# eladb3/SViT

Measured on AMD Instinct MI355X. Metric: clips/sec (fwd+bwd) SViT 16x224^2 bf16, higher is better.
Workload: dtype bf16; 1 GPU; SViT 16x224^2, 8 clips/GPU, 4 object tokens/frame, fwd+CE+bwd+clip+AdamW; global_batch=8, parallelism=dp1, ranks_seen=1, forced_dp=False, launch=hip-graph replay, input=fp32 clips, resident in the replayed step's input buffers, hip_library=svit_amd/lib/libsvit_hip.so

## Files before the change

### include/svit_hip.h

```cpp
#ifndef SVIT_HIP_H
#define SVIT_HIP_H
#include <stdint.h>
#ifdef __cplusplus
extern "C" {
#endif

#define SVIT_HEAD_DIM 96

int svit_version(void);
const char* svit_arch(void);

enum {
  SVIT_EPI_BF16 = 0,
  SVIT_EPI_GELU = 1,
  SVIT_EPI_RESID = 2,
  SVIT_EPI_F32 = 3,
  SVIT_EPI_DGELU = 4,
  SVIT_EPI_RELQ = 5
};
typedef struct {
  const void* A; int32_t lda;
  const void* W; int32_t ldw;
  const float* bias;
  void* out; int32_t ldo;
// ... 8 lines not shown
  int32_t relq_extra, relq_rows;
  float relq_scale;
} svit_gemm_args;
int svit_gemm_nt(const svit_gemm_args* args, void* stream);
int svit_gemm_tn(const void* A, int lda, const void* B, int ldb, float* dW, int lddw,
                 int M, int N, int K, int splits, float* dbias ,
                 void* stream);
#define SVIT_TN_GROUP_MAX 16
typedef struct {
  const void* A; const void* B; float* dW; float* dbias;
  int32_t lda, ldb, lddw, M, N, K;
} svit_tn_problem;
int svit_gemm_tn_grouped(const svit_tn_problem* probs, int count, void* stream);
int svit_gemm_tn_grouped_ex(const svit_tn_problem* probs, int count, int ordered, void* stream);
int svit_gemm_tn_grouped_slab(const svit_tn_problem* probs, int count, float* workspace,
                              int64_t workspace_floats, void* stream);
int64_t svit_gemm_tn_grouped_workspace(const svit_tn_problem* probs, int count);
int svit_colsum_bf16(const void* A, int lda, float* out, int M, int N, void* stream);

int svit_cast_f32_bf16(const float* src, void* dst, int64_t n, void* stream);
int svit_table_interp(const float* M, int rows, int J, const float* tables, float* out32, void* out16, void* stream);
typedef struct svit_table_interp_job {
  const float* M;
  const float* tables;
  float* out32;
  void* out16;
  int32_t rows, J;
} svit_table_interp_job;
int svit_table_interp_batched(const svit_table_interp_job* jobs_dev, int n_jobs, int max_rows, void* stream);
int svit_transpose_cast_batched(const float* src_base, void* dst_base, const int64_t* table,
                                int n_mats, int max_tiles, void* stream);
int svit_transpose_bf16_batched(const void* src_base, void* dst_base, const int64_t* table,
                                int n_mats, int max_tiles, void* stream);
int svit_pad_cast_rows(const float* src, void* dst, int R, int C, int ldd, void* stream);
int svit_scale_cast(const float* src, void* dst, const float* row_scale, int rows_per_sample,
                    int64_t rows, int cols, int gather_L, int gather_N, int gather_off,
                    void* stream);

int svit_reduce_defer(int on, void* stream);
int svit_reduce_flush(void* stream);
int svit_reduce_reset(void* stream);

int svit_layernorm_fwd(const float* x, const float* gamma, const float* beta, void* y_bf16,
                       float* y_f32, float* mean, float* rstd, int64_t rows, int C, float eps,
                       void* stream);
int svit_layernorm_bwd(const void* dy , int dy_is_bf16,
                       const float* x, const float* gamma, const float* mean,
                       const float* rstd, const float* dres, float* dx, void* dx_bf16,
                       const float* row_scale, int rows_per_sample, float* dgamma,
                       float* dbeta, int64_t rows, int C, float* workspace,
                       int64_t workspace_floats, void* stream);

int svit_im2col_patch(const float* video, void* cols, int B, int T, int H, int W, void* stream);
int svit_im2col_patch_u8(const uint8_t* frames, int64_t frames_bytes, const void* lut,
                         const int32_t* crops, void* cols, int B, int T, int Hs, int Ws, int S,
                         void* stream);
int svit_mixup_clips(float* x, const void* mix, int B, int planes, int H, int W, void* stream);
int svit_im2col_patch_u8_mix(const uint8_t* frames, int64_t frames_bytes, const float* lut_f32,
                             const int32_t* crops, const void* mix, void* cols, int B, int T, int Hs,
                             int Ws, int S, void* stream);
int svit_fill_special_tokens(float* x, const float* cls, const float* objq, const float* pos_t,
                             int B, int N, int L, int Tx, int O, int C, int add_pos, void* stream);
int svit_special_token_grads(const float* dx, float* g_cls, float* g_obj, float* g_pos, int B, int N,
                             int L, int Tx, int O, int C, int add_pos, void* stream);

typedef struct {
  const void* qkv; int32_t which;
  const float* conv_w;
  const float* gamma; const float* beta;
  void* out; int32_t ld_out;
  void* pre; float* mean; float* rstd;
  int32_t B, heads, T, H, W, n_obj;
  int32_t stride_hw;
  int32_t mode;
  float eps;
  float out_scale;
  const void* relq_R; const int32_t* relq_map; int32_t relq_lpad; float relq_scale;
} svit_pool_args;
int svit_pool_ln_fwd(const svit_pool_args* a, void* stream);

typedef struct {
  const void* d_main; int32_t main_is_f32; int32_t ld_main;
  const void* d_res; const void* d_extra;
  const void* pre; const float* mean; const float* rstd; const float* gamma;
  void* dpre; float* dgamma; float* dbeta;
  int32_t B, heads, Nout;
  float* workspace; int64_t workspace_floats;
  int32_t main_parts; int64_t main_part_stride;
  int32_t extra_is_bf16;
} svit_pool_ln_bwd_args;
int svit_pool_ln_bwd(const svit_pool_ln_bwd_args* a, void* stream);
typedef struct {
  const void* dpre; const float* conv_w; void* dqkv; int32_t which;
  int32_t B, heads, T, H, W, n_obj, stride_hw;
} svit_pool_dgrad_args;
typedef struct {
  const void* dpre; const void* qkv; int32_t which; float* dw;
  int32_t B, heads, T, H, W, n_obj, stride_hw;
  float* workspace; int64_t workspace_floats;
} svit_pool_wgrad_args;
int svit_pool_ln_fwd_qkv(const svit_pool_args* args3, void* stream);
int svit_pool_weight_sel(const float* src_base, const int64_t* src_off, uint32_t* dst, int n_tables,
                         void* stream);
int svit_pool_ln_fwd_qkv_sel(const svit_pool_args* args3, const uint32_t* const* sel3, void* stream);
int svit_pool_ln_bwd_qkv(const svit_pool_ln_bwd_args* args3, void* stream);
#ifdef SVIT_DIAG_POOL_STREAMING
// ... 127 lines not shown
```

### svit_amd/build.py

```python
import concurrent.futures
import os
import re
import subprocess
import sys

HERE = os.path.dirname(os.path.abspath(__file__))
CSRC = os.path.join(HERE, "csrc")
OUT_DIR = os.path.join(HERE, "lib")
LIB = os.path.join(OUT_DIR, "libsvit_hip.so")
SOURCES = ["gemm_nt.hip", "gemm_tn.hip", "norm.hip", "misc.hip", "pool.hip", "attn_fwd.hip", "attn_bwd.hip",
           "loss.hip", "meter.hip", "input.hip", "head.hip"]
HEADERS = ["common.h", "attn_common.h", "gemm_epilogue.h", os.path.join("..", "..", "include", "svit_hip.h")]
HIPCC = os.environ.get("HIPCC", "/opt/rocm/bin/hipcc")
FLAGS = ["--offload-arch=gfx950", "-O3", "-fPIC", "-std=c++17", "-ffast-math",
         "-fno-finite-math-only", "-fno-slp-vectorize", "-Wno-unused-result"]
TMP_DIR = os.path.join(OUT_DIR, "tmp")


_PK = re.compile(r"\s*(v_pk_(?:mul|add|fma)_f32)\s+v\[(\d+):\d+\],\s*(.*)")


def _sel(rest, name, n, default):
    m = re.search(name + r":\[([0-9,]+)\]", rest)
    v = [int(x) for x in m.group(1).split(",")] if m else []
    return v + [default] * (n - len(v))


def hazardous_packed_f32(asm_text):
    bad = []
    for ln, line in enumerate(asm_text.splitlines(), 1):
        m = _PK.match(line)
        if not m:
            continue
        rest = m.group(3).split("//")[0]
        ops = [o.strip() for o in re.split(r",\s*(?![^\[]*\])", rest.split(" op_sel")[0].split(" neg_")[0])]
        sel = _sel(rest, "op_sel", len(ops), 0) if re.search(r"op_sel:\[", rest) else [0] * len(ops)
        sel_hi = _sel(rest, "op_sel_hi", len(ops), 1)
        for i, o in enumerate(ops):
            if re.match(r"v\[(\d+):\d+\]", o) and (sel[i] == 1 or sel_hi[i] == 0):
                bad.append((ln, line.split("//")[0].strip()))
                break
    return bad


LLVM_OBJDUMP = os.environ.get("LLVM_OBJDUMP", "/opt/rocm/lib/llvm/bin/llvm-objdump")


def disassemble(lib=None):
    import shutil
    import tempfile
    lib = lib or LIB
    tmp = tempfile.mkdtemp(prefix="svit_isa_")
    try:
        cp = os.path.join(tmp, "lib.so")
        shutil.copy(lib, cp)
        r = subprocess.run([LLVM_OBJDUMP, "--offloading", cp], capture_output=True, text=True, cwd=tmp)
        if r.returncode != 0:
            raise RuntimeError("llvm-objdump --offloading failed: %s" % r.stderr[-300:])
        objs = sorted(f for f in os.listdir(tmp) if "amdgcn" in f and "gfx950" in f)
        text = []
        for f in objs:
            d = subprocess.run([LLVM_OBJDUMP, "-d", "--no-show-raw-insn", os.path.join(tmp, f)],
                               capture_output=True, text=True)
            if d.returncode != 0:
# ... 69 lines not shown
```

### svit_amd/engine.py

```python
import math

import torch

from . import arch, hip, ops
from .input import U8Clips

HD = arch.HEAD_DIM
F32, BF16 = torch.float32, torch.bfloat16
SCALE = HD ** -0.5
LOG2E = 1.4426950408889634
K_SCALE = SCALE * LOG2E


def _align(n, a=8):
    return (n + a - 1) // a * a


class FlatParams:

    def __init__(self, shapes, decay_of, device, rank_of):
        names = list(shapes)
        depth = 1 + max([int(n.split(".")[1]) for n in names if n.startswith("blocks.")] or [0])
        ranks = {n: rank_of(n, depth) for n in names}
        order = sorted(names, key=lambda n: (not decay_of(n, shapes[n]), ranks[n]))
# ... 83 lines not shown

    def sels(self, pre):
        return [self.pool_sel[self.pool_sel_index[pre + "attn.pool_%s.weight" % r]] for r in "qkv"]

    TILED_MIN_PLANE = 2048
    SLAB_MAX_PLANE = 196

    def refresh_low_precision(self):
        ops.cast_bf16(self.data, self.w16[:self.total])
        if self.pool_sel_index:
            ops.pool_weight_sel(self.data, self.pool_sel_off, self.pool_sel)
        if self.n_t:
            ops.transpose_bf16_batched(self.w16, self.wT16, self.t_table, self.n_t, 256)


def rel_sections(rows):
    off_w = _align(rows[0])
    off_t = off_w + _align(rows[1])
    return (0, off_w, off_t), _align(off_t + rows[2], 32)


def _rel_index(q_n, k_n):
    q_ratio = max(k_n / q_n, 1.0)
    k_ratio = max(q_n / k_n, 1.0)
    d = torch.arange(q_n)[:, None] * q_ratio - torch.arange(k_n)[None, :] * k_ratio
    d = d + (k_n - 1) * k_ratio
    return d.long().to(torch.int32)


def _resize_matrix(rows_have, rows_need):
    m = torch.zeros(rows_need, rows_have)
    scale = rows_have / rows_need
    for i in range(rows_need):
        pos = max((i + 0.5) * scale - 0.5, 0.0)
        i0 = min(int(math.floor(pos)), rows_have - 1)
        i1 = min(i0 + 1, rows_have - 1)
        lam = pos - i0
        m[i, i0] += 1.0 - lam
        m[i, i1] += lam
    return m


class Engine:
    def __init__(self, plan: arch.Plan, flat: FlatParams, red_group=4):
        self.plan, self.flat = plan, flat
        self.dev = flat.data.device
        self._rel_cache = {}
        self._interp_cache = {}
        self._interp_out = {}
        self.batch_interp = True
        self._relq_cache = {}
        self.fused_scatter = True
        self.patch_w16 = torch.zeros((plan.embed_dim, 448), device=self.dev, dtype=BF16)
        self._tn = []
        self.RED_GROUP = max(1, int(red_group))
        M1 = 1024 * 1024
        self._red_ws = torch.empty(self.RED_GROUP * 18 * M1, device=self.dev, dtype=F32)
        self._red_slot = 0
        self._wgrad_need, self._wgrad_big = {}, {}
        self._red_regions = {"ln2": (0, 4 * M1), "ln1": (4 * M1, 8 * M1), "pln": (8 * M1, 9 * M1),
                             "wgrad": (9 * M1, 18 * M1)}
        self._side = None
        self._side_keep = []
        self._side_active = False
        self.overlap_wgrad = False
        self.attn_q_splits = 0
        self.deterministic = False
        self.reproducible = False
        self._capture_fork = None
        self._capture_join = None

    def refresh_weights(self):
        self.flat.refresh_low_precision()
        ops.pad_cast_rows(self.flat.p("patch_embed.proj.weight").view(self.plan.embed_dim, 441),
                          self.patch_w16)

    def _rel(self, blk, q_thw, k_thw):
        key = (blk.index, q_thw, k_thw)
        ent = self._rel_cache.get(key)
        if ent is None:
            idx = [_rel_index(q_thw[1], k_thw[1]), _rel_index(q_thw[2], k_thw[2]),
                   _rel_index(q_thw[0], k_thw[0])]
            need = [2 * max(q_thw[i], k_thw[i]) - 1 for i in (1, 2, 0)]
            have = [blk.rel_sp_rows, blk.rel_sp_rows, blk.rel_t_rows]
            mats = [None if n == h else _resize_matrix(h, n).to(self.dev) for n, h in zip(need, have)]
            mcat = None
            if any(m is not None for m in mats):
                lp = (sum(need) + 95) // 96 * 96
                mcat = torch.zeros((lp, sum(have)), device=self.dev)
                r0 = c0 = 0
                for n, h, m in zip(need, have, mats):
                    mcat[r0:r0 + n, c0:c0 + h] = torch.eye(h, device=self.dev) if m is None else m
                    r0, c0 = r0 + n, c0 + h
            ent = ([t.contiguous().to(self.dev) for t in idx], mats, mcat, tuple(need))
            self._rel_cache[key] = ent
        return ent

    def _interp_tables(self, thw, save):
        if not self.batch_interp:
            self._interp_out = {}
            return
        key = (tuple(thw), bool(save))
        ent = self._interp_cache.get(key)
        if ent is None:
            entries, outs, cur = [], {}, tuple(thw)
            for blk in self.plan.blocks:
                sq, skv = blk.stride_q[1], blk.stride_kv[1]
                q_thw = (cur[0], arch.pooled(cur[1], sq), arch.pooled(cur[2], sq))
                k_thw = (cur[0], arch.pooled(cur[1], skv), arch.pooled(cur[2], skv))
                _, _, mcat, _ = self._rel(blk, q_thw, k_thw)
                if mcat is not None:
                    r32 = torch.empty((mcat.shape[0], HD), device=self.dev, dtype=F32) if save else None
                    r16 = torch.empty((mcat.shape[0], HD), device=self.dev, dtype=BF16)
                    entries.append((mcat, self.flat.rel_tables32("blocks.%d." % blk.index), r32, r16))
                    outs[blk.index] = (r32, r16)
                cur = q_thw
            jobs = ops.table_interp_jobs(entries, self.dev) if entries else None
            ent = (jobs, max((e[0].shape[0] for e in entries), default=0), outs, entries)
            self._interp_cache[key] = ent
        jobs, max_rows, outs, _ = ent
        if jobs is not None:
            ops.table_interp_batched(jobs, max_rows)
        self._interp_out = outs

    def _relq_map(self, blk, q_thw, k_thw, idx, rows_off, n_obj, extra):
        key = (blk.index, q_thw, k_thw, tuple(rows_off), n_obj, extra)
        m = self._relq_cache.get(key)
        if m is None:
            qt, qh, qw = q_thw
            kt, kh, kw = k_thw
            ih, iw, it = (t.cpu().view(n, k) for t, n, k in zip(idx, (qh, qw, qt), (kh, kw, kt)))
            Lq = qt * qh * qw
            body = torch.full((qt, qh, qw, extra), -1, dtype=torch.int32)
            body[..., :kh] = (rows_off[0] + ih).view(1, qh, 1, kh)
            body[..., kh:kh + kw] = (rows_off[1] + iw).view(1, 1, qw, kw)
            body[..., kh + kw:kh + kw + kt] = (rows_off[2] + it).view(qt, 1, 1, kt)
            m = torch.full((1 + Lq + n_obj, extra), -1, dtype=torch.int32)
            m[1:1 + Lq] = body.view(Lq, extra)
            m = m.contiguous().to(self.dev)
            self._relq_cache[key] = m
        return m

    def _tables(self, pre, mats):
        names = (pre + "attn.rel_pos_h", pre + "attn.rel_pos_w", pre + "attn.rel_pos_t")
        out = []
        for n, m in zip(names, mats):
            t = self.flat.p(n)
            out.append(t if m is None else (m @ t).contiguous())
        return out

    def forward(self, video, drop_scales=None, save=True):
        plan, f = self.plan, self.flat
        if isinstance(video, U8Clips):
            B, _, Tx = video.shape[:3]
            cols, (To, Ho, Wo) = ops.im2col_patch_u8(video)
        else:
            if video.dim() == 4:
                video = video.unsqueeze(2)
            video = video.contiguous().to(F32)
            B, _, Tx = video.shape[:3]
            cols, (To, Ho, Wo) = ops.im2col_patch(video)
        T = plan.num_frames // plan.patch_stride[0] if Tx > 1 else Tx
        if To != T:
            raise hip.SvitHipError("clip has %d frames but cfg.DATA.NUM_FRAMES=%d" % (Tx, plan.num_frames))
        L, n_obj, C = To * Ho * Wo, Tx * plan.objects, plan.embed_dim
        N = 1 + L + n_obj
        x = torch.empty((B, N, C), device=self.dev, dtype=F32)
        ops.gemm_nt(cols, self.patch_w16, f.p("patch_embed.proj.bias"), hip.EPI_F32,
                    out=x.view(B * N, C), remap=(L, N, 1))
        ops.fill_special_tokens(x, f.p("cls_token"), f.p("object_queries"),
                                f.p("pos_embed_temporal"), L, Tx, plan.objects, Tx > 1)
        st = {"B": B, "Tx": Tx, "n_obj": n_obj, "L0": L, "cols": cols if save else None,
              "blocks": []}
        thw = (T, Ho, Wo)
        self._interp_tables(thw, save)
        hip.mark("stem")
        for blk in plan.blocks:
            ds = drop_scales[blk.index] if drop_scales is not None else None
            x, thw, sv = self._block_fwd(blk, x, thw, n_obj, ds, save)
            st["blocks"].append(sv)
            hip.mark("fwd%d" % blk.index)
        y16, y32, mean, rstd = ops.layernorm_fwd(x, f.p("norm.weight"), f.p("norm.bias"),
                                                 want_f32=True, want_bf16=False, save_stats=save)
        st.update(x_last=x if save else None, mean=mean, rstd=rstd, thw=thw)
        self._interp_out = {}
        return y32, st

    def _block_fwd(self, blk, x, thw, n_obj, ds, save):
        f = self.flat
        pre = "blocks.%d." % blk.index
        B, N, C = x.shape
        Co, h = blk.dim_out, blk.heads
        sq, skv = blk.stride_q[1], blk.stride_kv[1]
        q_thw = (thw[0], arch.pooled(thw[1], sq), arch.pooled(thw[2], sq))
        k_thw = (thw[0], arch.pooled(thw[1], skv), arch.pooled(thw[2], skv))
        Nq = 1 + q_thw[0] * q_thw[1] * q_thw[2] + n_obj
        J = k_thw[0] + k_thw[1] + k_thw[2]
        DA = HD + 32 if J <= 32 else HD + 64
        if J > 64:
            raise hip.SvitHipError("key grid %s too large for the in-MFMA rel-pos bias" % (k_thw,))
        xn, _, mean1, rstd1 = ops.layernorm_fwd(x, f.p(pre + "norm1.weight"), f.p(pre + "norm1.bias"),
                                                save_stats=save)
        xn2d = xn.view(B * N, C)
        qkv = ops.gemm_nt(xn2d, f.w(pre + "attn.qkv.weight"), f.p(pre + "attn.qkv.bias"), hip.EPI_BF16)
        idx, mats, mcat, need = self._rel(blk, q_thw, k_thw)
        if mcat is None:
            tabs = self._tables(pre, mats)
            rcat, rows_off = f.rel_cat(pre)
        else:
            if blk.index in self._interp_out:
                r32, rcat = self._interp_out[blk.index]
            else:
                r32, rcat = ops.table_interp(mcat, f.rel_tables32(pre), want_f32=save)
            rows_off = (0, need[0], need[0] + need[1])
            tabs = None if r32 is None else [r32[rows_off[0]:rows_off[0] + need[0]], r32[rows_off[1]:rows_off[1] + need[1]],
                                             r32[rows_off[2]:rows_off[2] + need[2]]]
        pools = ops.pool_ln_fwd_qkv(
            qkv, [f.p(pre + "attn.pool_%s.weight" % r).view(HD, 27) for r in "qkv"],
            [f.p(pre + "attn.norm_%s.weight" % r) for r in "qkv"],
            [f.p(pre + "attn.norm_%s.bias" % r) for r in "qkv"],
            B, h, thw, n_obj, (sq, skv, skv), (DA, DA, HD), (0, 1, 0), save=save, out_scales=(1.0, K_SCALE, 1.0),
            sels=f.sels(pre) if (thw[1] * thw[2] >= f.TILED_MIN_PLANE or thw[1] * thw[2] <= f.SLAB_MAX_PLANE)
            else None,
            relq=(rcat.contiguous(), self._relq_map(blk, q_thw, k_thw, idx, rows_off, n_obj, DA - HD), LOG2E))
        qa, ka, v = pools[0][0], pools[1][0], pools[2][0]
        ctx, lse2 = ops.attn_fwd(qa, ka, v, SCALE, bias_cols=J)
# ... 6 lines not shown
        if blk.pools_q:
            skip, pool_idx = ops.maxpool_fwd(skip, thw, n_obj)
        dpa, dpm = ds if ds is not None else (None, None)
        x1 = ops.gemm_nt(ctx.view(B * Nq, Co), f.w(pre + "attn.proj.weight"), f.p(pre + "attn.proj.bias"),
                         hip.EPI_RESID, aux=skip.view(B * Nq, Co), row_scale=dpa, rows_per_sample=Nq)
        x1 = x1.view(B, Nq, Co)
        xn2, _, mean2, rstd2 = ops.layernorm_fwd(x1, f.p(pre + "norm2.weight"), f.p(pre + "norm2.bias"),
                                                 save_stats=save)
        act, dact = ops.gemm_nt(xn2.view(B * Nq, Co), f.w(pre + "mlp.fc1.weight"),
                                f.p(pre + "mlp.fc1.bias"), hip.EPI_GELU, save=save)
        x2 = ops.gemm_nt(act, f.w(pre + "mlp.fc2.weight"), f.p(pre + "mlp.fc2.bias"), hip.EPI_RESID,
                         aux=x1.view(B * Nq, Co), row_scale=dpm, rows_per_sample=Nq).view(B, Nq, Co)
        sv = None
        if save:
            sv = dict(x=x, thw=thw, q_thw=q_thw, k_thw=k_thw, mean1=mean1, rstd1=rstd1, xn=xn2d,
                      qkv=qkv, pools=pools, tabs=tabs, idx=idx, mats=mats, ctx=ctx, lse2=lse2,
                      pool_idx=pool_idx, x1=x1, mean2=mean2, rstd2=rstd2, xn2=xn2, act=act,
                      dact=dact, dpa=dpa, dpm=dpm, Nq=Nq)
        return x2, q_thw, sv

    def backward(self, st, dy, on_ready=None, ready_ranks=None):
        def ready(rank):
            if on_ready is not None:
                if ready_ranks is None or rank in ready_ranks:
                    ops.reduce_flush()
                    self._flush_tn()
                    self._join()
                on_ready(rank)
        plan, f = self.plan, self.flat
        depth = len(plan.blocks)
        last = st["blocks"][depth - 1]
        dx, dx16 = ops.layernorm_bwd(dy.contiguous(), st["x_last"], f.p("norm.weight"), st["mean"],
                                     st["rstd"], f.g("norm.weight"), f.g("norm.bias"),
                                     want_bf16=True, row_scale=last["dpm"],
                                     rows_per_sample=st["x_last"].shape[1])
        ready(0)
        hip.mark("bwd_norm")
        for blk in reversed(plan.blocks):
            below = st["blocks"][blk.index - 1] if blk.index > 0 else None
            try:
                G = self.RED_GROUP
                dx, dx16 = self._block_bwd(blk, st["blocks"][blk.index], dx, dx16, st["n_obj"], below,
                                           red_begin=blk.index % G == G - 1 or blk.index == depth - 1,
                                           red_end=blk.index % G == 0, red_slot=blk.index % G)
            except BaseException:
                ops.reduce_reset()
                self._tn = []
                raise
            hip.mark("bwd%d" % blk.index)
            ready(1 + (depth - 1 - blk.index))
        B, Tx, L, O, C = st["B"], st["Tx"], st["L0"], plan.objects, plan.embed_dim
        ops.special_token_grads(dx, f.g("cls_token"), f.g("object_queries"),
                                f.g("pos_embed_temporal") if Tx > 1 else None, L, Tx, O, Tx > 1)
        dtok = ops.scale_cast(dx, gather=(L, 1))
        self._gemm_tn(dtok, st["cols"], f.g("patch_embed.proj.weight").view(C, 441), f.g("patch_embed.proj.bias"))
        self._flush_tn()
        self._join()
        ready(depth + 1)

    def _rws(self, key):
        a, b = self._red_regions[key]
        o = self._red_slot * 18 * 1024 * 1024
        return self._red_ws[o + a:o + b]

    def _wgrad_ws(self, B, h, thw, n_obj, strides):
        key = (B, h, tuple(thw), n_obj, tuple(strides))
        need = self._wgrad_need.get(key)
        if need is None:
            need = self._wgrad_need[key] = ops.pool_conv_bwd_workspace(B, h, thw, n_obj, strides)
        ws = self._rws("wgrad")
        if need <= ws.numel():
            return ws
        big = self._wgrad_big.get(self._red_slot)
        if big is None or big.numel() < need:
            big = self._wgrad_big[self._red_slot] = torch.empty(need, device=self.dev, dtype=F32)
        return big

    def _fork(self, fn, keep):
        if not self.overlap_wgrad:
            fn()
            return
        if self._capture_fork is not None:
            self._capture_fork(fn)
            self._side_active = True
            return
        main = torch.cuda.current_stream(self.dev)
        if self._side is None:
            self._side = torch.cuda.Stream(device=self.dev)
        self._side.wait_stream(main)
        with torch.cuda.stream(self._side):
            fn()
        self._side_keep.append(keep)
        self._side_active = True

    def _join(self):
        if self._side_active and self._capture_join is not None:
            self._capture_join()
            self._side_active = False
            return
        if self._side_active:
            torch.cuda.current_stream(self.dev).wait_stream(self._side)
            self._side_keep.clear()
            self._side_active = False

    def _flush_tn(self, force=True):
        if not force and len(self._tn) <= 8:
            return
        q, self._tn = self._tn, []
# ... 123 lines not shown
```

### svit_amd/hip.py

```python
import ctypes as C
import os

import torch

_HERE = os.path.dirname(os.path.abspath(__file__))
LIB_PATH = os.environ.get("SVIT_HIP_LIB") or os.path.join(_HERE, "lib", "libsvit_hip.so")
_lib = None

vp, i32, i64, f32 = C.c_void_p, C.c_int32, C.c_int64, C.c_float

EPI_BF16, EPI_GELU, EPI_RESID, EPI_F32, EPI_DGELU, EPI_RELQ = 0, 1, 2, 3, 4, 5


class TnProblem(C.Structure):
    _fields_ = [("A", vp), ("B", vp), ("dW", vp), ("dbias", vp), ("lda", i32), ("ldb", i32),
                ("lddw", i32), ("M", i32), ("N", i32), ("K", i32)]


class GemmArgs(C.Structure):
    _fields_ = [("A", vp), ("lda", i32), ("W", vp), ("ldw", i32), ("bias", vp), ("out", vp),
                ("ldo", i32), ("out2", vp), ("ldo2", i32), ("aux", vp), ("ldaux", i32),
                ("row_scale", vp), ("rows_per_sample", i32), ("M", i32), ("N", i32), ("K", i32),
                ("epilogue", i32), ("accumulate", i32), ("remap_L", i32), ("remap_N", i32),
                ("remap_off", i32), ("relq_map", vp), ("relq_out", vp), ("relq_ld", i32),
# ... 59 lines not shown


class AttnFwdArgs(C.Structure):
    _fields_ = [("qa", vp), ("ka", vp), ("v", vp), ("ctx", vp), ("lse2", vp), ("B", i32),
                ("heads", i32), ("Nq", i32), ("Nk", i32), ("DA", i32), ("scale", f32),
                ("bias_cols", i32)]


class AttnBwdArgs(C.Structure):
    _fields_ = [("qa", vp), ("ka", vp), ("v", vp), ("ctx", vp), ("dctx", vp), ("lse2", vp),
                ("delta", vp), ("dqa", vp), ("dk", vp), ("dv", vp), ("B", i32), ("heads", i32),
                ("Nq", i32), ("Nk", i32), ("DA", i32), ("q_splits", i32), ("scale", f32),
                ("bias_cols", i32), ("relD", vp), ("relD_ld", i32), ("relD_map", vp), ("relD_scale", f32),
                ("relR", vp), ("relX", vp)]


class HeadArgs(C.Structure):
    _fields_ = [("tokens", vp), ("B", i32), ("N", i32), ("C", i32), ("T", i32), ("O", i32), ("keep", vp),
                ("w_proj", vp), ("b_proj", vp), ("n_cls", i32), ("w_box", vp), ("b_box", vp),
                ("w_bce", vp), ("b_bce", vp), ("w_con", vp), ("b_con", vp),
                ("logits", vp), ("boxes", vp), ("contact", vp), ("xobj", vp)]


class HeadBwdArgs(C.Structure):
    _fields_ = [("f", HeadArgs), ("dlogits", vp), ("dboxes", vp), ("dcontact", vp), ("dxobj", vp), ("dtokens", vp),
                ("gw_proj", vp), ("gb_proj", vp), ("gw_box", vp), ("gb_box", vp), ("gw_bce", vp), ("gb_bce", vp),
                ("gw_con", vp), ("gb_con", vp), ("ordered", i32)]


_SIGS = {
    "svit_version": (i32, []),
    "svit_arch": (C.c_char_p, []),
    "svit_gemm_nt": (i32, [C.POINTER(GemmArgs), vp]),
    "svit_gemm_tn": (i32, [vp, i32, vp, i32, vp, i32, i32, i32, i32, i32, vp, vp]),
    "svit_gemm_tn_grouped": (i32, [C.POINTER(TnProblem), i32, vp]),
    "svit_gemm_tn_grouped_ex": (i32, [C.POINTER(TnProblem), i32, i32, vp]),
    "svit_gemm_tn_grouped_slab": (i32, [C.POINTER(TnProblem), i32, vp, i64, vp]),
    "svit_gemm_tn_grouped_workspace": (i64, [C.POINTER(TnProblem), i32]),
    "svit_colsum_bf16": (i32, [vp, i32, vp, i32, i32, vp]),
    "svit_cast_f32_bf16": (i32, [vp, vp, i64, vp]),
    "svit_table_interp": (i32, [vp, i32, i32, vp, vp, vp, vp]),
    "svit_table_interp_batched": (i32, [vp, i32, i32, vp]),
    "svit_transpose_cast_batched": (i32, [vp, vp, vp, i32, i32, vp]),
    "svit_transpose_bf16_batched": (i32, [vp, vp, vp, i32, i32, vp]),
    "svit_scale_cast": (i32, [vp, vp, vp, i32, i64, i32, i32, i32, i32, vp]),
    "svit_pad_cast_rows": (i32, [vp, vp, i32, i32, i32, vp]),
    "svit_reduce_defer": (i32, [i32, vp]),
    "svit_reduce_flush": (i32, [vp]),
    "svit_reduce_reset": (i32, [vp]),
    "svit_layernorm_fwd": (i32, [vp, vp, vp, vp, vp, vp, vp, i64, i32, f32, vp]),
    "svit_layernorm_bwd": (i32, [vp, i32, vp, vp, vp, vp, vp, vp, vp, vp, i32, vp, vp, i64, i32, vp,
                                 i64, vp]),
    "svit_im2col_patch": (i32, [vp, vp, i32, i32, i32, i32, vp]),
    "svit_im2col_patch_u8": (i32, [vp, i64, vp, vp, vp, i32, i32, i32, i32, i32, vp]),
    "svit_im2col_patch_u8_mix": (i32, [vp, i64, vp, vp, vp, vp, i32, i32, i32, i32, i32, vp]),
    "svit_mixup_clips": (i32, [vp, vp, i32, i32, i32, i32, vp]),
    "svit_fill_special_tokens": (i32, [vp, vp, vp, vp, i32, i32, i32, i32, i32, i32, i32, vp]),
    "svit_special_token_grads": (i32, [vp, vp, vp, vp, i32, i32, i32, i32, i32, i32, i32, vp]),
    "svit_pool_ln_fwd": (i32, [C.POINTER(PoolArgs), vp]),
    "svit_pool_ln_bwd": (i32, [C.POINTER(PoolLnBwdArgs), vp]),
    "svit_pool_ln_fwd_qkv": (i32, [C.POINTER(PoolArgs), vp]),
    "svit_pool_ln_fwd_qkv_sel": (i32, [C.POINTER(PoolArgs), C.POINTER(vp), vp]),
    "svit_pool_weight_sel": (i32, [vp, vp, vp, i32, vp]),
    "svit_pool_ln_bwd_qkv": (i32, [C.POINTER(PoolLnBwdArgs), vp]),
    "svit_pool_conv_bwd_qkv": (i32, [C.POINTER(PoolDgradArgs), C.POINTER(PoolWgradArgs), vp]),
    "svit_pool_conv_bwd_workspace": (i64, [C.POINTER(PoolDgradArgs)]),
    "svit_relpos_q_fwd": (i32, [C.POINTER(RelqArgs), vp]),
    "svit_relpos_q_bwd": (i32, [C.POINTER(RelqBwdArgs), vp]),
    "svit_relpos_scatter": (i32, [C.POINTER(RelqScatterArgs), vp]),
    "svit_relpos_gather": (i32, [C.POINTER(RelqGatherArgs), vp]),
    "svit_attn_fwd": (i32, [C.POINTER(AttnFwdArgs), vp]),
    "svit_attn_bwd": (i32, [C.POINTER(AttnBwdArgs), vp]),
    "svit_attn_bwd_parts": (i32, [C.POINTER(AttnBwdArgs)]),
    "svit_maxpool_fwd": (i32, [vp, vp, vp, i32, i32, i32, i32, i32, i32, vp]),
    "svit_maxpool_bwd": (i32, [vp, vp, vp, i32, i32, i32, i32, i32, i32, vp]),
    "svit_maxpool_bwd_bf16": (i32, [vp, vp, vp, i32, i32, i32, i32, i32, i32, vp]),
    "svit_sumsq": (i32, [vp, i64, vp, vp, i64, vp]),
    "svit_adamw_step": (i32, [vp, vp, vp, vp, i64, vp, f32, f32, f32, f32, f32, f32, i32, f32, vp]),
    "svit_head_fwd": (i32, [C.POINTER(HeadArgs), vp]),
    "svit_head_bwd": (i32, [C.POINTER(HeadBwdArgs), vp]),
    "svit_haog_loss": (i32, [vp, vp, vp, vp, vp, vp, vp, vp, vp, i32, i32, vp]),
    "svit_haog_loss_bwd": (i32, [vp, vp, vp, vp, vp, vp, vp, i32, i32, vp]),
    "svit_ce_loss": (i32, [vp, vp, i32, i32, vp, vp, vp]),
    "svit_ce_loss_soft": (i32, [vp, vp, vp, vp, f32, f32, i32, i32, vp, vp, vp]),
    "svit_step_draws": (i32, [vp, vp, i32, i32, vp, i32, C.c_float, vp, vp]),
    "svit_ensemble_update": (i32, [vp, vp, vp, i32, i32, i32, i32, i32, i32, vp, vp, vp, vp, vp]),
    "svit_topk_correct": (i32, [vp, vp, i32, i32, vp, i32, vp, vp, vp]),
    "svit_debug_set": (i32, [i32, i32]),
    "svit_debug_set_tn": (i32, [i32, i32]),
    "svit_debug_set_tn_tile": (i32, [i32]),
    "svit_debug_set_pool": (i32, [i32, i32]),
    "svit_attn_debug_set": (i32, [i32, i32]),
    "svit_debug_reset": (i32, []),
    "svit_debug_pool_bwd_path": (i32, []),
}
EXPORTS = tuple(sorted(_SIGS))


class SvitHipError(RuntimeError):
    pass


def load():
    global _lib
    if _lib is None:
        if not os.path.exists(LIB_PATH):
# ... 70 lines not shown
```

### svit_amd/ops.py

```python
import ctypes as C

import torch

from . import hip
from .hip import ptr

BF16 = torch.bfloat16
F32 = torch.float32
HD = 96
_scratch = {}


def scratch(device, floats=8 * 1024 * 1024, tag="main"):
    key = (device.index, floats, tag)
    buf = _scratch.get(key)
    if buf is None:
        buf = torch.empty(floats, device=device, dtype=F32)
        _scratch[key] = buf
    return buf


def _chk_rows(*ts):
    for t in ts:
        if not t.is_cuda or t.dim() != 2 or t.stride(1) != 1:
# ... 226 lines not shown
        shape = src.shape
    else:
        gl, go = gather
        gn = src.shape[-2]
        rows = src.shape[0] * gl
        shape = (rows, cols)
    if dst is None:
        dst = torch.empty(shape, device=src.device, dtype=BF16)
    hip.call("svit_scale_cast", ptr(src), ptr(dst), ptr(row_scale), rows_per_sample, rows, cols,
             gl, gn, go)
    return dst


def layernorm_fwd(x, gamma, beta, eps=1e-6, want_f32=False, want_bf16=True, save_stats=True):
    _chk_dev(x, gamma, beta)
    C_ = x.shape[-1]
    rows = x.numel() // C_
    y16 = torch.empty(x.shape, device=x.device, dtype=BF16) if want_bf16 else None
    y32 = torch.empty(x.shape, device=x.device, dtype=F32) if want_f32 else None
    mean = torch.empty(rows, device=x.device, dtype=F32) if save_stats else None
    rstd = torch.empty(rows, device=x.device, dtype=F32) if save_stats else None
    hip.call("svit_layernorm_fwd", ptr(x), ptr(gamma), ptr(beta), ptr(y16), ptr(y32), ptr(mean),
             ptr(rstd), rows, C_, eps)
    return y16, y32, mean, rstd


def layernorm_bwd(dy, x, gamma, mean, rstd, dgamma, dbeta, dres=None, dx=None, want_bf16=False,
                  row_scale=None, rows_per_sample=0, ws=None):
    _chk_dev(dy, x, gamma, mean, rstd, dgamma, dbeta, dres, dx, row_scale)
    C_ = x.shape[-1]
    rows = x.numel() // C_
    if dx is None:
        dx = torch.empty(x.shape, device=x.device, dtype=F32)
    dx16 = torch.empty(x.shape, device=x.device, dtype=BF16) if want_bf16 else None
    ws = scratch(x.device) if ws is None else ws
    assert dy.dtype in (F32, BF16)
    hip.call("svit_layernorm_bwd", ptr(dy), int(dy.dtype == BF16), ptr(x), ptr(gamma), ptr(mean),
             ptr(rstd), ptr(dres),
             ptr(dx), ptr(dx16), ptr(row_scale), rows_per_sample, ptr(dgamma), ptr(dbeta), rows, C_,
             ptr(ws), ws.numel())
    return (dx, dx16) if want_bf16 else dx


def im2col_patch(video):
    _chk_dev(video)
    B, Cin, T, H, W = video.shape
    assert Cin == 3 and video.dtype == F32
    To, Ho, Wo = (T - 1) // 2 + 1, (H - 1) // 4 + 1, (W - 1) // 4 + 1
    cols = torch.empty((B * To * Ho * Wo, 448), device=video.device, dtype=BF16)
    hip.call("svit_im2col_patch", ptr(video), ptr(cols), B, T, H, W)
    return cols, (To, Ho, Wo)


def im2col_patch_u8(clips):
    fr = clips.frames
    _chk_dev(fr)
    V, T, Hs, Ws, _ = fr.shape
    B, S = clips.crops.shape[0], clips.size
    To, Ho, Wo = (T - 1) // 2 + 1, (S - 1) // 4 + 1, (S - 1) // 4 + 1
    cols = torch.empty((B * To * Ho * Wo, 448), device=fr.device, dtype=BF16)
    mix = getattr(clips, "mix", None)
    if mix is not None:
        _chk_mix(mix, fr.device)
        hip.call("svit_im2col_patch_u8_mix", ptr(fr), fr.numel(), ptr(clips.lut_f32), ptr(clips.crops), ptr(mix),
                 ptr(cols), B, T, Hs, Ws, S)
        return cols, (To, Ho, Wo)
    hip.call("svit_im2col_patch_u8", ptr(fr), fr.numel(), ptr(clips.lut), ptr(clips.crops),
             ptr(cols), B, T, Hs, Ws, S)
    return cols, (To, Ho, Wo)


def _chk_mix(mix, device):
    _chk_dev(mix)
    if mix.dtype != torch.int32 or mix.numel() != 8 or mix.device != device:
        raise hip.SvitHipError("the mix record must be int32 [8] on %s (got %s %s on %s)"
                               % (device, mix.dtype, tuple(mix.shape), mix.device))


def mixup_clips(x, mix):
    _chk_dev(x)
    _chk_mix(mix, x.device)
    if x.dtype != F32 or x.dim() < 3:
        raise hip.SvitHipError("mixup_clips needs an fp32 [B, ..., H, W] tensor, got %s %s" % (x.dtype, tuple(x.shape)))
    B, H, W = x.shape[0], x.shape[-2], x.shape[-1]
    hip.call("svit_mixup_clips", ptr(x), ptr(mix), B, x[0].numel() // (H * W), H, W)
    return x


def fill_special_tokens(x, cls, objq, pos_t, L, Tx, O, add_pos):
    B, N, C_ = x.shape
    hip.call("svit_fill_special_tokens", ptr(x), ptr(cls), ptr(objq), ptr(pos_t), B, N, L, Tx, O,
             C_, int(add_pos))


def special_token_grads(dx, g_cls, g_obj, g_pos, L, Tx, O, add_pos):
    B, N, C_ = dx.shape
    assert dx.is_contiguous() and dx.dtype == F32
    hip.call("svit_special_token_grads", ptr(dx), ptr(g_cls), ptr(g_obj), ptr(g_pos), B, N, L, Tx, O, C_, int(add_pos))


def pooled(n, s):
    return (n - 1) // s + 1


NOGRAD_SCRATCH = True

# ... 378 lines not shown
```

Baseline: 699.6 clips/s.

## Fuse patch-embed conv into implicit-GEMM kernels reading fp32 video directly

```diff
diff --git a/include/svit_hip.h b/include/svit_hip.h
--- a/include/svit_hip.h
+++ b/include/svit_hip.h
@@ -84,6 +84,12 @@
                        int64_t workspace_floats, void* stream);
 
 int svit_im2col_patch(const float* video, void* cols, int B, int T, int H, int W, void* stream);
+int svit_patch_embed_grid(void);
+int64_t svit_patch_embed_wgrad_workspace(void);
+int svit_patch_embed_fwd(const float* video, const void* w16p, const float* bias, float* x, int B, int T, int H, int W,
+                         int N, void* stream);
+int svit_patch_embed_wgrad(const float* video, const float* dx, float* dw, float* dbias, int B, int T, int H, int W,
+                           int N, float* workspace, int64_t workspace_floats, void* stream);
 int svit_im2col_patch_u8(const uint8_t* frames, int64_t frames_bytes, const void* lut,
                          const int32_t* crops, void* cols, int B, int T, int Hs, int Ws, int S,
                          void* stream);
diff --git a/svit_amd/build.py b/svit_amd/build.py
--- a/svit_amd/build.py
+++ b/svit_amd/build.py
@@ -9,7 +9,7 @@
 OUT_DIR = os.path.join(HERE, "lib")
 LIB = os.path.join(OUT_DIR, "libsvit_hip.so")
 SOURCES = ["gemm_nt.hip", "gemm_tn.hip", "norm.hip", "misc.hip", "pool.hip", "attn_fwd.hip", "attn_bwd.hip",
-           "loss.hip", "meter.hip", "input.hip", "head.hip"]
+           "loss.hip", "meter.hip", "input.hip", "head.hip", "stem.hip"]
 HEADERS = ["common.h", "attn_common.h", "gemm_epilogue.h", os.path.join("..", "..", "include", "svit_hip.h")]
 HIPCC = os.environ.get("HIPCC", "/opt/rocm/bin/hipcc")
 FLAGS = ["--offload-arch=gfx950", "-O3", "-fPIC", "-std=c++17", "-ffast-math",
diff --git a/svit_amd/csrc/stem.hip b/svit_amd/csrc/stem.hip
--- /dev/null
+++ b/svit_amd/csrc/stem.hip
@@ -0,0 +1,304 @@
+#include "common.h"
+#include "../../include/svit_hip.h"
+
+namespace {
+
+typedef unsigned u32x4_t __attribute__((ext_vector_type(4)));
+
+constexpr int PE_GRID = 256;
+constexpr int PE_XO = 64;
+constexpr int PE_SLOTS = PE_XO + 1;
+constexpr int PE_PITCH = 288;
+constexpr int PE_IMG = 64 * PE_PITCH;
+constexpr int PE_WLD = 63 * 8;
+constexpr int PE_SLAB = 96 * 441 + 96;
+constexpr int FWD_NT = 256, FWD_NPF = (63 * PE_SLOTS + FWD_NT - 1) / FWD_NT;
+constexpr int WG_NT = 512, WG_NPF = (63 * PE_SLOTS + WG_NT - 1) / WG_NT;
+constexpr int FWD_LDS = 2 * PE_IMG * 2;
+constexpr int WG_DT = 64 * 96;
+constexpr int WG_LDS = 2 * PE_IMG * 2 + 2 * WG_DT * 2;
+
+struct PeGeom {
+  int B, T, H, W, To, Ho, Wo, nchunks, items, per;
+};
+
+template <int NT, int NPF>
+__device__ __forceinline__ uint64_t pe_issue(const float* __restrict__ video, const PeGeom& g, int item, int tid,
+                                             u32x4_t (&pf)[NPF]) {
+  const int line = item / g.nchunks, chunk = item - line * g.nchunks;
+  const int yo = line % g.Ho, tb = line / g.Ho, to = tb % g.To, b = tb / g.To;
+  const size_t clip = (size_t)3 * g.T * g.H * g.W;
+  const auto rs = __builtin_amdgcn_make_buffer_rsrc((void*)(video + (size_t)b * clip), 0, (int)(clip * 4), 0x00020000);
+  uint64_t m = 0;
+#pragma unroll
+  for (int j = 0; j < NPF; ++j) {
+    const int i = tid + NT * j, r = i / PE_SLOTS, s = i - r * PE_SLOTS;
+    const int ky = r % 7, kt = (r / 7) % 3, c = r / 21;
+    const int t = to * 2 - 1 + kt, y = yo * 4 - 3 + ky, x0 = (chunk * PE_XO + s) * 4 - 3;
+    const bool row_ok = r < 63 && t >= 0 && t < g.T && y >= 0 && y < g.H && x0 < g.W;
+    const int xl = x0 < 0 ? 0 : min(x0, g.W - 4);
+    const int off = row_ok ? (((c * g.T + t) * g.H + y) * g.W + xl) * 4 : 0;
+    pf[j] = __builtin_amdgcn_raw_buffer_load_b128(rs, off, 0, 0);
+    unsigned bits = 0;
+#pragma unroll
+    for (int e = 0; e < 4; ++e) bits |= (unsigned)(row_ok && x0 + e >= 0 && x0 + e < g.W) << e;
+    m |= (uint64_t)bits << (4 * j);
+  }
+  return m;
+}
+
+template <int NT, int NPF>
+__device__ __forceinline__ void pe_write(bf16_t* __restrict__ img, int tid, const u32x4_t (&pf)[NPF], uint64_t m) {
+#pragma unroll
+  for (int j = 0; j < NPF; ++j) {
+    const int i = tid + NT * j, r = i / PE_SLOTS, s = i - r * PE_SLOTS;
+    if (i < 63 * PE_SLOTS) {
+      const unsigned bits = (unsigned)(m >> (4 * j)) & 15u;
+      const float a0 = __uint_as_float(pf[j].x), a1 = __uint_as_float(pf[j].y);
+      const float a2 = __uint_as_float(pf[j].z), a3 = __uint_as_float(pf[j].w);
+      float v0 = a0, v1 = a1, v2 = a2, v3 = a3;
+      if (bits == 8u) v3 = a0;
+      else if (bits == 7u) { v0 = a1; v1 = a2; v2 = a3; }
+      else if (bits == 3u) { v0 = a2; v1 = a3; }
+      else if (bits == 1u) v0 = a3;
+      v0 = (bits & 1) ? v0 : 0.f; v1 = (bits & 2) ? v1 : 0.f;
+      v2 = (bits & 4) ? v2 : 0.f; v3 = (bits & 8) ? v3 : 0.f;
+      uint2 pk;
+      pk.x = pack_bf16x2(v0, v1); pk.y = pack_bf16x2(v2, v3);
+      *(uint2*)(img + r * PE_PITCH + s * 4) = pk;
+    }
+  }
+}
+
+__device__ __forceinline__ uint2 pe_ld8(const bf16_t* p) {
+  typedef __attribute__((address_space(3))) uint64_t lds_u64_t;
+  const uint64_t v = *(const volatile lds_u64_t*)(__attribute__((address_space(3))) void*)p;
+  return make_uint2((uint32_t)v, (uint32_t)(v >> 32));
+}
+
+__device__ __forceinline__ bf16x8_t pe_frag(uint2 lo, uint2 hi) {
+  const uint4 u = make_uint4(lo.x, lo.y, hi.x, hi.y);
+  return __builtin_bit_cast(bf16x8_t, u);
+}
+
+__global__ __launch_bounds__(FWD_NT) void patch_embed_fwd_kernel(const float* __restrict__ video,
+                                                                 const bf16_t* __restrict__ w16p,
+                                                                 const float* __restrict__ bias, float* __restrict__ x,
+                                                                 const PeGeom g, int N) {
+  extern __shared__ __attribute__((aligned(16))) unsigned char pe_lds[];
+  bf16_t* img = (bf16_t*)pe_lds;
+  const int tid = threadIdx.x, lane = tid & 63, wave = __builtin_amdgcn_readfirstlane(tid >> 6);
+  const int nt = min(wave, 2), hh = lane >> 5, ln = lane & 31;
+  const int start = blockIdx.x * g.per, end = min(start + g.per, g.items);
+  if (start >= end) return;
+  for (int i = tid; i < 2 * PE_PITCH; i += FWD_NT)
+    img[(i / PE_PITCH) * PE_IMG + 63 * PE_PITCH + i % PE_PITCH] = 0;
+  const int ch = nt * 32 + ln;
+  bf16x8_t bw[32];
+#pragma unroll
+  for (int s = 0; s < 32; ++s) {
+    uint4 u = make_uint4(0u, 0u, 0u, 0u);
+    if (s < 31 || hh == 0) u = *(const uint4*)(w16p + (size_t)ch * PE_WLD + s * 16 + hh * 8);
+    bw[s] = __builtin_bit_cast(bf16x8_t, u);
+  }
+  const float bias_v = bias ? bias[ch] : 0.f;
+
+  u32x4_t pf[FWD_NPF];
+  uint64_t m = pe_issue<FWD_NT, FWD_NPF>(video, g, start, tid, pf);
+  pe_write<FWD_NT, FWD_NPF>(img, tid, pf, m);
+  __syncthreads();
+  for (int item = start; item < end; ++item) {
+    const int cur = (item - start) & 1;
+    const bool more = item + 1 < end;
+    if (more) m = pe_issue<FWD_NT, FWD_NPF>(video, g, item + 1, tid, pf);
+    if (wave < 3) {
+      const bf16_t* a = img + cur * PE_IMG + hh * PE_PITCH + ln * 4;
+      f32x16_t acc0, acc1;
+#pragma unroll
+      for (int r = 0; r < 16; ++r) acc0[r] = acc1[r] = 0.f;
+#pragma unroll
+      for (int s = 0; s < 32; ++s) {
+        const uint2 l0 = pe_ld8(a + (2 * s) * PE_PITCH), h0 = pe_ld8(a + (2 * s) * PE_PITCH + 4);
+        const uint2 l1 = pe_ld8(a + (2 * s) * PE_PITCH + 128), h1 = pe_ld8(a + (2 * s) * PE_PITCH + 132);
+        acc0 = mfma32(pe_frag(l0, h0), bw[s], acc0);
+        acc1 = mfma32(pe_frag(l1, h1), bw[s], acc1);
+      }
+      const int line = item / g.nchunks, chunk = item - line * g.nchunks;
+      const int b = line / (g.Ho * g.To), lrow = line - b * g.Ho * g.To;
+      float* out = x + ((size_t)b * N + 1 + (size_t)lrow * g.Wo) * 96 + ch;
+#pragma unroll
+      for (int r = 0; r < 16; ++r) {
+        const int xo = chunk * PE_XO + acc_row(r, lane);
+        if (xo < g.Wo) out[(size_t)xo * 96] = acc0[r] + bias_v;
+        if (xo + 32 < g.Wo) out[(size_t)(xo + 32) * 96] = acc1[r] + bias_v;
+      }
+    }
+    if (more) pe_write<FWD_NT, FWD_NPF>(img + (cur ^ 1) * PE_IMG, tid, pf, m);
+    __syncthreads();
+  }
+}
+
+__global__ __launch_bounds__(WG_NT) void patch_embed_wgrad_kernel(const float* __restrict__ video,
+                                                                  const float* __restrict__ dx, float* __restrict__ slab,
+                                                                  const PeGeom g, int N) {
+  extern __shared__ __attribute__((aligned(16))) unsigned char pe_lds[];
+  bf16_t* img = (bf16_t*)pe_lds;
+  bf16_t* dt = img + 2 * PE_IMG;
+  const int tid = threadIdx.x, lane = tid & 63, wave = __builtin_amdgcn_readfirstlane(tid >> 6);
+  const int start = blockIdx.x * g.per, end = min(start + g.per, g.items);
+  if (start >= end) return;
+  for (int i = tid; i < 2 * PE_PITCH; i += WG_NT)
+    img[(i / PE_PITCH) * PE_IMG + 63 * PE_PITCH + i % PE_PITCH] = 0x3F80;
+
+  auto dt_issue = [&](int item, float4 (&df)[3]) -> unsigned {
+    const int line = item / g.nchunks, chunk = item - line * g.nchunks;
+    const int b = line / (g.Ho * g.To), lrow = line - b * g.Ho * g.To;
+    const int n_xo = min(PE_XO, g.Wo - chunk * PE_XO);
+    const float* src = dx + ((size_t)b * N + 1 + (size_t)lrow * g.Wo + chunk * PE_XO) * 96;
+    unsigned ok = 0;
+#pragma unroll
+    for (int j = 0; j < 3; ++j) {
+      const int i = tid + WG_NT * j, tok = i / 24, c4 = i - tok * 24;
+      df[j] = *(const float4*)(src + (size_t)min(tok, n_xo - 1) * 96 + c4 * 4);
+      ok |= (unsigned)(tok < n_xo) << j;
+    }
+    return ok;
+  };
+  auto dt_write = [&](bf16_t* d, const float4 (&df)[3], unsigned ok) {
+#pragma unroll
+    for (int j = 0; j < 3; ++j) {
+      const int i = tid + WG_NT * j;
+      uint2 pk = make_uint2(0u, 0u);
+      if ((ok >> j) & 1) { pk.x = pack_bf16x2(df[j].x, df[j].y); pk.y = pack_bf16x2(df[j].z, df[j].w); }
+      *(uint2*)(d + i * 4) = pk;
+    }
+  };
+
+  const int hh = lane >> 5, cg = (lane >> 4) & 1, ii = lane & 15, q = ii >> 2, pp = ii & 3;
+  int a_off[3], b_off[2];
+#pragma unroll
+  for (int i = 0; i < 3; ++i) a_off[i] = (8 * hh + q) * 96 + i * 32 + 16 * cg + 4 * pp;
+#pragma unroll
+  for (int j = 0; j < 2; ++j)
+    b_off[j] = (4 * (2 * wave + j) + 2 * cg + (pp >> 1)) * PE_PITCH + (8 * hh + q) * 4 + 4 * (pp & 1);
+
+  f32x16_t acc[3][2];
+#pragma unroll
+  for (int i = 0; i < 3; ++i)
+#pragma unroll
+    for (int j = 0; j < 2; ++j)
+#pragma unroll
+      for (int r = 0; r < 16; ++r) acc[i][j][r] = 0.f;
+
+  u32x4_t pf[WG_NPF];
+  float4 df[3];
+  uint64_t m = pe_issue<WG_NT, WG_NPF>(video, g, start, tid, pf);
+  unsigned ok = dt_issue(start, df);
+  pe_write<WG_NT, WG_NPF>(img, tid, pf, m);
+  dt_write(dt, df, ok);
+  __syncthreads();
+  for (int item = start; item < end; ++item) {
+    const int cur = (item - start) & 1;
+    const bool more = item + 1 < end;
+    if (more) {
+      m = pe_issue<WG_NT, WG_NPF>(video, g, item + 1, tid, pf);
+      ok = dt_issue(item + 1, df);
+    }
+    const bf16_t* ia = img + cur * PE_IMG;
+    const bf16_t* da = dt + cur * WG_DT;
+#pragma unroll
+    for (int ks = 0; ks < 4; ++ks) {
+      bf16x8_t fa[3], fb[2];
+#pragma unroll
+      for (int i = 0; i < 3; ++i)
+        fa[i] = make_bf16x8(lds_read_tr16(da + a_off[i] + ks * 16 * 96), lds_read_tr16(da + a_off[i] + (ks * 16 + 4) * 96));
+#pragma unroll
+      for (int j = 0; j < 2; ++j)
+        fb[j] = make_bf16x8(lds_read_tr16(ia + b_off[j] + ks * 64), lds_read_tr16(ia + b_off[j] + ks * 64 + 16));
+#pragma unroll
+      for (int i = 0; i < 3; ++i)
+#pragma unroll
+        for (int j = 0; j < 2; ++j) acc[i][j] = mfma32(fa[i], fb[j], acc[i][j]);
+    }
+    if (more) {
+      pe_write<WG_NT, WG_NPF>(img + (cur ^ 1) * PE_IMG, tid, pf, m);
+      dt_write(dt + (cur ^ 1) * WG_DT, df, ok);
+    }
+    __syncthreads();
+  }
+  float* out = slab + (size_t)blockIdx.x * PE_SLAB;
+#pragma unroll
+  for (int j = 0; j < 2; ++j) {
+    const int kp = 32 * (2 * wave + j) + (lane & 31), r_img = kp >> 3, kx = kp & 7;
+#pragma unroll
+    for (int i = 0; i < 3; ++i)
+#pragma unroll
+      for (int r = 0; r < 16; ++r) {
+        const int c = i * 32 + acc_row(r, lane);
+        if (r_img < 63 && kx < 7) out[c * 441 + r_img * 7 + kx] = acc[i][j][r];
+        else if (kp == 504) out[96 * 441 + c] = acc[i][j][r];
+      }
+  }
+}
+
+SvitOnce g_fwd_once, g_wgrad_once;
+
+int pe_geom(PeGeom* g, int B, int T, int H, int W) {
+  if (B <= 0 || T <= 0 || H <= 0 || W <= 0) return SVIT_ERR_ARG;
+  if (W < 4) return SVIT_ERR_SHAPE;
+  if ((int64_t)3 * T * H * W * 4 >= (1ll << 31)) return SVIT_ERR_SHAPE;
+  g->B = B; g->T = T; g->H = H; g->W = W;
+  g->To = (T + 2 - 3) / 2 + 1; g->Ho = (H + 6 - 7) / 4 + 1; g->Wo = (W + 6 - 7) / 4 + 1;
+  g->nchunks = (g->Wo + PE_XO - 1) / PE_XO;
+  const int64_t items = (int64_t)B * g->To * g->Ho * g->nchunks;
+  if (items >= (1ll << 31)) return SVIT_ERR_SHAPE;
+  g->items = (int)items;
+  g->per = (g->items + PE_GRID - 1) / PE_GRID;
+  return SVIT_OK;
+}
+
+}
+
+extern "C" int svit_patch_embed_grid(void) { return PE_GRID; }
+
+extern "C" int64_t svit_patch_embed_wgrad_workspace(void) { return (int64_t)PE_GRID * PE_SLAB; }
+
+extern "C" int svit_patch_embed_fwd(const float* video, const void* w16p, const float* bias, float* x, int B, int T,
+                                    int H, int W, int N, void* stream) {
+  if (!video || !w16p || !x) return SVIT_ERR_ARG;
+  PeGeom g;
+  const int rc = pe_geom(&g, B, T, H, W);
+  if (rc) return rc;
+  if (N < 1 + g.To * g.Ho * g.Wo) return SVIT_ERR_SHAPE;
+  if (((uintptr_t)video & 3) || ((uintptr_t)w16p & 15)) return SVIT_ERR_ALIGN;
+  const int e = svit_max_lds_once(g_fwd_once, (const void*)patch_embed_fwd_kernel, FWD_LDS);
+  if (e) return e;
+  const int grid = (g.items + g.per - 1) / g.per;
+  hipLaunchKernelGGL(patch_embed_fwd_kernel, dim3(grid), dim3(FWD_NT), FWD_LDS, (hipStream_t)stream, video,
+                     (const bf16_t*)w16p, bias, x, g, N);
+  SVIT_LAUNCH_CHECK();
+  return SVIT_OK;
+}
+
+extern "C" int svit_patch_embed_wgrad(const float* video, const float* dx, float* dw, float* dbias, int B, int T, int H,
+                                      int W, int N, float* workspace, int64_t workspace_floats, void* stream) {
+  if (!video || !dx || !dw || !dbias || !workspace) return SVIT_ERR_ARG;
+  PeGeom g;
+  const int rc = pe_geom(&g, B, T, H, W);
+  if (rc) return rc;
+  if (N < 1 + g.To * g.Ho * g.Wo) return SVIT_ERR_SHAPE;
+  if (((uintptr_t)video & 3) || ((uintptr_t)dx & 15)) return SVIT_ERR_ALIGN;
+  const int grid = (g.items + g.per - 1) / g.per;
+  if (workspace_floats < (int64_t)grid * PE_SLAB) return SVIT_ERR_ARG;
+  const int e = svit_max_lds_once(g_wgrad_once, (const void*)patch_embed_wgrad_kernel, WG_LDS);
+  if (e) return e;
+  hipLaunchKernelGGL(patch_embed_wgrad_kernel, dim3(grid), dim3(WG_NT), WG_LDS, (hipStream_t)stream, video, dx,
+                     workspace, g, N);
+  SVIT_LAUNCH_CHECK();
+  SvitReduceDst dst;
+  dst.ptr[0] = dw; dst.end[0] = 96 * 441;
+  for (int k = 1; k < 6; ++k) { dst.ptr[k] = dbias; dst.end[k] = PE_SLAB; }
+  svit_launch_reduce(workspace, grid, PE_SLAB, dst, (hipStream_t)stream);
+  SVIT_LAUNCH_CHECK();
+  return SVIT_OK;
+}
diff --git a/svit_amd/engine.py b/svit_amd/engine.py
--- a/svit_amd/engine.py
+++ b/svit_amd/engine.py
@@ -159,6 +159,8 @@
         self._relq_cache = {}
         self.fused_scatter = True
         self.patch_w16 = torch.zeros((plan.embed_dim, 448), device=self.dev, dtype=BF16)
+        self.fused_stem = "auto"
+        self.patch_w16p = torch.zeros((plan.embed_dim, 63 * 8), device=self.dev, dtype=BF16)
         self._tn = []
         self.RED_GROUP = max(1, int(red_group))
         M1 = 1024 * 1024
@@ -181,6 +183,19 @@
         self.flat.refresh_low_precision()
         ops.pad_cast_rows(self.flat.p("patch_embed.proj.weight").view(self.plan.embed_dim, 441),
                           self.patch_w16)
+        ops.patch_embed_pack_weight(self.flat.p("patch_embed.proj.weight"), self.patch_w16p)
+
+    def _stem_is_fused(self, video, save):
+        mode = self.fused_stem
+        if mode not in ("auto", "always", "never"):
+            raise hip.SvitHipError("engine.fused_stem must be 'auto', 'always' or 'never' (got %r)" % (mode,))
+        if mode == "never" or isinstance(video, U8Clips):
+            return False
+        if mode == "always" or not save:
+            return True
+        if self.deterministic or self.reproducible:
+            return False
+        return ops.patch_embed_lines(video) >= ops.patch_embed_grid()
 
     def _rel(self, blk, q_thw, k_thw):
         key = (blk.index, q_thw, k_thw)
@@ -258,6 +273,8 @@
 
     def forward(self, video, drop_scales=None, save=True):
         plan, f = self.plan, self.flat
+        fused = self._stem_is_fused(video, save)
+        cols = None
         if isinstance(video, U8Clips):
             B, _, Tx = video.shape[:3]
             cols, (To, Ho, Wo) = ops.im2col_patch_u8(video)
@@ -266,19 +283,25 @@
                 video = video.unsqueeze(2)
             video = video.contiguous().to(F32)
             B, _, Tx = video.shape[:3]
-            cols, (To, Ho, Wo) = ops.im2col_patch(video)
+            if fused:
+                To, Ho, Wo = (Tx - 1) // 2 + 1, (video.shape[3] - 1) // 4 + 1, (video.shape[4] - 1) // 4 + 1
+            else:
+                cols, (To, Ho, Wo) = ops.im2col_patch(video)
         T = plan.num_frames // plan.patch_stride[0] if Tx > 1 else Tx
         if To != T:
             raise hip.SvitHipError("clip has %d frames but cfg.DATA.NUM_FRAMES=%d" % (Tx, plan.num_frames))
         L, n_obj, C = To * Ho * Wo, Tx * plan.objects, plan.embed_dim
         N = 1 + L + n_obj
         x = torch.empty((B, N, C), device=self.dev, dtype=F32)
-        ops.gemm_nt(cols, self.patch_w16, f.p("patch_embed.proj.bias"), hip.EPI_F32,
-                    out=x.view(B * N, C), remap=(L, N, 1))
+        if fused:
+            ops.patch_embed_fwd(video, self.patch_w16p, f.p("patch_embed.proj.bias"), x)
+        else:
+            ops.gemm_nt(cols, self.patch_w16, f.p("patch_embed.proj.bias"), hip.EPI_F32,
+                        out=x.view(B * N, C), remap=(L, N, 1))
         ops.fill_special_tokens(x, f.p("cls_token"), f.p("object_queries"),
                                 f.p("pos_embed_temporal"), L, Tx, plan.objects, Tx > 1)
         st = {"B": B, "Tx": Tx, "n_obj": n_obj, "L0": L, "cols": cols if save else None,
-              "blocks": []}
+              "video": video if (save and fused) else None, "blocks": []}
         thw = (T, Ho, Wo)
         self._interp_tables(thw, save)
         hip.mark("stem")
@@ -391,8 +414,12 @@
         B, Tx, L, O, C = st["B"], st["Tx"], st["L0"], plan.objects, plan.embed_dim
         ops.special_token_grads(dx, f.g("cls_token"), f.g("object_queries"),
                                 f.g("pos_embed_temporal") if Tx > 1 else None, L, Tx, O, Tx > 1)
-        dtok = ops.scale_cast(dx, gather=(L, 1))
-        self._gemm_tn(dtok, st["cols"], f.g("patch_embed.proj.weight").view(C, 441), f.g("patch_embed.proj.bias"))
+        if st.get("video") is not None:
+            ops.patch_embed_wgrad(st["video"], dx, f.g("patch_embed.proj.weight").view(C, 441),
+                                  f.g("patch_embed.proj.bias"))
+        else:
+            dtok = ops.scale_cast(dx, gather=(L, 1))
+            self._gemm_tn(dtok, st["cols"], f.g("patch_embed.proj.weight").view(C, 441), f.g("patch_embed.proj.bias"))
         self._flush_tn()
         self._join()
         ready(depth + 1)
diff --git a/svit_amd/hip.py b/svit_amd/hip.py
--- a/svit_amd/hip.py
+++ b/svit_amd/hip.py
@@ -135,6 +135,10 @@
     "svit_layernorm_bwd": (i32, [vp, i32, vp, vp, vp, vp, vp, vp, vp, vp, i32, vp, vp, i64, i32, vp,
                                  i64, vp]),
     "svit_im2col_patch": (i32, [vp, vp, i32, i32, i32, i32, vp]),
+    "svit_patch_embed_grid": (i32, []),
+    "svit_patch_embed_wgrad_workspace": (i64, []),
+    "svit_patch_embed_fwd": (i32, [vp, vp, vp, vp, i32, i32, i32, i32, i32, vp]),
+    "svit_patch_embed_wgrad": (i32, [vp, vp, vp, vp, i32, i32, i32, i32, i32, vp, i64, vp]),
     "svit_im2col_patch_u8": (i32, [vp, i64, vp, vp, vp, i32, i32, i32, i32, i32, vp]),
     "svit_im2col_patch_u8_mix": (i32, [vp, i64, vp, vp, vp, vp, i32, i32, i32, i32, i32, vp]),
     "svit_mixup_clips": (i32, [vp, vp, i32, i32, i32, i32, vp]),
diff --git a/svit_amd/ops.py b/svit_amd/ops.py
--- a/svit_amd/ops.py
+++ b/svit_amd/ops.py
@@ -302,6 +302,45 @@
     return cols, (To, Ho, Wo)
 
 
+def patch_embed_pack_weight(w, out=None):
+    _chk_dev(w, out)
+    if out is None:
+        out = torch.empty((96, 504), device=w.device, dtype=BF16)
+    pad_cast_rows(w.view(96 * 63, 7), out.view(96 * 63, 8))
+    return out
+
+
+def patch_embed_lines(video):
+    B, _, T, H, _ = video.shape
+    return B * ((T - 1) // 2 + 1) * ((H - 1) // 4 + 1)
+
+
+def patch_embed_grid():
+    return hip.load().svit_patch_embed_grid()
+
+
+def patch_embed_fwd(video, w16p, bias, x):
+    _chk_dev(video, w16p, bias, x)
+    B, Cin, T, H, W = video.shape
+    assert Cin == 3 and video.dtype == F32 and x.dtype == F32 and w16p.dtype == BF16 and w16p.shape == (96, 504)
+    To, Ho, Wo = (T - 1) // 2 + 1, (H - 1) // 4 + 1, (W - 1) // 4 + 1
+    assert x.shape[0] == B and x.shape[2] == 96 and x.shape[1] >= 1 + To * Ho * Wo
+    hip.call("svit_patch_embed_fwd", ptr(video), ptr(w16p), ptr(bias), ptr(x), B, T, H, W, x.shape[1],
+             meta=("bytes", video.numel() * 4 + B * To * Ho * Wo * 96 * 4))
+    return To, Ho, Wo
+
+
+def patch_embed_wgrad(video, dx, dw, dbias):
+    _chk_dev(video, dx, dw, dbias)
+    B, Cin, T, H, W = video.shape
+    assert Cin == 3 and video.dtype == F32 and dx.dtype == F32 and dw.dtype == F32 and dbias.dtype == F32
+    assert dw.numel() == 96 * 441 and dbias.numel() == 96 and dx.shape[0] == B and dx.shape[2] == 96
+    ws = scratch(video.device, floats=hip.load().svit_patch_embed_wgrad_workspace(), tag="patch_wgrad")
+    hip.call("svit_patch_embed_wgrad", ptr(video), ptr(dx), ptr(dw), ptr(dbias), B, T, H, W, dx.shape[1],
+             ptr(ws), ws.numel(), meta=("bytes", video.numel() * 4 + dx.numel() * 4))
+    return dw
+
+
 def im2col_patch_u8(clips):
     fr = clips.frames
     _chk_dev(fr)
```

New measurement: 701.8 clips/s (median of 6 runs). Within noise of the previous version (+0.3%).
